# Complexity-ML/complexity-tokenizer

Hardware: AMD Instinct MI355X
Metric: MB/s raw UTF-8 encoded (encode_batch), 50k ByteLevel BPE, 1/2/4/8 MI355X (higher is better)
Workload: dtype u8

## Files before the change

complexity-tokenizer_amd/complexity_tokenizer/__init__.py:

```python
from __future__ import annotations

import ctypes
import gc
import os

import numpy as np

from . import _native as _n
from . import _fast

__version__ = "0.3.3"
__all__ = ["Tokenizer", "Trainer", "BpeTrainer", "WordPieceTrainer", "WordPieceModel", "UnigramTrainer", "UnigramModel", "Encoding",
           "BatchEncoding", "PanicException", "UnsupportedConfigError", "DeviceError", "__version__"]


class PanicException(BaseException):
    """Raised where the reference raises pyo3_runtime.PanicException (a Rust panic), e.g. a
    merge rank that indexes past the list of valid merges (reference src/bpe.rs:141)."""


class UnsupportedConfigError(NotImplementedError):
    """tokenizer.json selects a component outside the ByteLevel-BPE encode path."""


# ... 204 lines not shown
        return buf.raw[:n.value].decode("utf-8")

    @property
    def special_tokens(self) -> dict:
        out = {}
        for i in range(int(_n.lib.ctok_num_special_tokens(self._h))):
            n = ctypes.c_size_t()
            tid = ctypes.c_uint32()
            buf = ctypes.create_string_buffer(1024)
            rc = _n.lib.ctok_special_token(self._h, i, buf, 1024, ctypes.byref(n), ctypes.byref(tid))
            if rc != _n.CTOK_OK:
                _raise(rc)
            if n.value > 1024:
                buf = ctypes.create_string_buffer(n.value)
                _n.lib.ctok_special_token(self._h, i, buf, n.value, ctypes.byref(n), ctypes.byref(tid))
            out[buf.raw[:n.value].decode("utf-8")] = int(tid.value)
        return out

    def num_piece_added_tokens(self) -> int:
        return int(_n.lib.ctok_num_piece_added_tokens(self._h))

    @property
    def table_props(self) -> dict:
        tp = _n.TableProps(dev_mid_packed=-1)
        rc = _n.lib.ctok_get_table_props(self._h, int(self.device), ctypes.byref(tp))
        if rc != _n.CTOK_OK:
            _raise(rc)
        d = {k: None if getattr(tp, k) < 0 else bool(getattr(tp, k)) for k, _ in tp._fields_}
        d["dev_mid_packed"] = None if tp.dev_mid_packed < 0 else int(tp.dev_mid_packed)
        return d

    def encode_packed(self, text: np.ndarray, off: np.ndarray, timing: bool = False):
        text = np.ascontiguousarray(text, dtype=np.uint8)
        off = np.ascontiguousarray(off, dtype=np.uint64)
        n_docs = len(off) - 1
        if n_docs < 0:
            raise ValueError("offsets must hold n_docs + 1 entries")
        n_bytes = int(off[-1]) if n_docs >= 0 else 0
        if len(text) < n_bytes:
            raise ValueError("text shorter than offsets[-1]")
        cap = int(n_bytes + n_docs + 16)
        while True:
            ids = np.empty(max(cap, 1), dtype=np.uint32)
            tok_off = np.empty(n_docs + 1, dtype=np.uint64)
            ex = self._host_exec(timing)
            st = _n.Stats()
            rc = _n.lib.ctok_encode_batch(self._h, text.ctypes.data, off.ctypes.data, n_docs, ids.ctypes.data, cap,
                                          tok_off.ctypes.data, ctypes.byref(ex), ctypes.byref(st))
            if rc == _n.CTOK_E_CAPACITY:
                cap = int(tok_off[-1])
                continue
            if rc != _n.CTOK_OK:
# ... 470 lines not shown
```

complexity-tokenizer_amd/complexity_tokenizer/_native.py:

```python
from __future__ import annotations

import ctypes
import os

_HERE = os.path.dirname(os.path.abspath(__file__))
LIB_PATH = os.environ.get("CTOK_LIB", os.path.join(_HERE, "libctok.so"))

if not os.path.exists(LIB_PATH):
    raise ImportError(
        "complexity_tokenizer: native library not found at %s -- build it with "
        "`make -C complexity-tokenizer_amd/csrc` (or `python -c 'import __graft_entry__ as g; g.build()'`)" % LIB_PATH)


def _share_torch_hip_runtime():
    if os.environ.get("CTOK_NO_TORCH_HIP"):
        return
    try:
        import importlib.util
        spec = importlib.util.find_spec("torch")
    except (ImportError, ValueError):
        return
    if spec is None or not spec.origin:
        return
    path = os.path.join(os.path.dirname(spec.origin), "lib", "libamdhip64.so")
# ... 61 lines not shown
CTOK_P_PAD_LONGEST = 8
CTOK_P_PAD_TO_MAX = 16
CTOK_P_PAD_LEFT = 32
CTOK_P_PAD_ID = 64
CTOK_P_NO_POSTPROCESS = 128
CTOK_P_WINDOWS = 256
CTOK_PP_SEQUENCE = 0xFFFFFFFF


class PadOpts(ctypes.Structure):
    _fields_ = [("flags", ctypes.c_uint32), ("pad_id", ctypes.c_uint32), ("max_length", ctypes.c_uint64)]


class Tables(ctypes.Structure):
    _fields_ = [("vocab", ctypes.c_char_p), ("vocab_off", ctypes.c_void_p), ("vocab_id", ctypes.c_void_p),
                ("n_vocab", ctypes.c_uint64), ("merge_left", ctypes.c_void_p), ("merge_right", ctypes.c_void_p),
                ("n_merges", ctypes.c_uint64), ("added", ctypes.c_char_p), ("added_off", ctypes.c_void_p),
                ("added_id", ctypes.c_void_p), ("added_flags", ctypes.c_void_p), ("n_added", ctypes.c_uint64),
                ("nfc", ctypes.c_int), ("add_prefix_space", ctypes.c_int)]


class TableProps(ctypes.Structure):
    _fields_ = [(k, ctypes.c_int) for k in ("narrow", "compact", "short_packed", "ids16", "dev_narrow",
                                            "dev_short_packed", "last_rec16", "last_wire16", "dev_mid_packed")]


class TrainerConfig(ctypes.Structure):
    _fields_ = [("vocab_size", ctypes.c_uint64), ("min_frequency", ctypes.c_uint32),
                ("min_word_length", ctypes.c_uint64), ("inl_alpha", ctypes.c_float), ("inl_beta", ctypes.c_float),
                ("inl_gate", ctypes.c_float), ("inl_mu_target", ctypes.c_float),
                ("inl_velocity_max", ctypes.c_float), ("inl_beta_max", ctypes.c_float),
                ("special", ctypes.c_char_p), ("special_off", ctypes.POINTER(ctypes.c_uint64)),
                ("n_special", ctypes.c_uint64), ("device", ctypes.c_int)]


class TrainerCountStats(ctypes.Structure):
    _fields_ = [("pieces", ctypes.c_uint64), ("words", ctypes.c_uint64), ("unique_words", ctypes.c_uint64),
                ("chunks", ctypes.c_uint64), ("host_chunks", ctypes.c_uint64), ("rerun_chunks", ctypes.c_uint64),
                ("bytes_d2h", ctypes.c_uint64), ("ms_device", ctypes.c_double), ("ms_host", ctypes.c_double)]


class BpeTrainerConfig(ctypes.Structure):
    _fields_ = [("vocab_size", ctypes.c_uint64), ("min_frequency", ctypes.c_uint32),
                ("special", ctypes.c_char_p), ("special_off", ctypes.POINTER(ctypes.c_uint64)),
                ("n_special", ctypes.c_uint64), ("end_of_word_suffix", ctypes.c_char_p),
                ("continuing_subword_prefix", ctypes.c_char_p), ("show_progress", ctypes.c_int),
                ("device", ctypes.c_int)]
# ... 160 lines not shown
```

complexity-tokenizer_amd/csrc/ctok_encode.cpp:

```cpp
#include <chrono>
#include <cstdio>
#include <cstring>

#include "call_plan.h"
#include "gen/unicode_data.h"
#include "host_internal.h"
#include "knobs.h"

ctok::ctok() = default;
ctok::~ctok() = default;

namespace ctok_rt __attribute__((visibility("hidden"))) {

bool cp_fast_ok() {
  static const bool ok = [] {
    if (process_knobs().no_cp_ranges) return false;
    for (uint32_t cp = 0x3000; cp < 0x1F700; cp++) {
      const int rc = cp_range_class(cp);
      if (rc < 0) continue;
      const int cl = (ct_cls_stage2[ct_cls_stage1[cp >> 8] * 64 + ((cp & 255) >> 2)] >> ((cp & 3) * 2)) & 3;
      if (cl != rc || ct_nfc_stage2[ct_nfc_stage1[cp >> 8] * 256 + (cp & 255)] != 0) return false;
    }
    return true;
  }();
// ... 90 lines not shown
  tb.decomp_off = ds->decomp_off.p;
  tb.decomp_data = ds->decomp_data.p;
  tb.n_decomp = CT_DECOMP_N;
  tb.comp_key = ds->comp_key.p;
  tb.comp_val = ds->comp_val.p;
  tb.n_comp = CT_COMP_N;
  tb.bytemap_alnum = ds->alnum.p;
  tb.at_bytes = ds->at_bytes.p;
  tb.at_off = ds->at_off.p;
  tb.at_id = ds->at_id.p;
  tb.at_flags = ds->at_flags.p;
  tb.n_at = (uint32_t)t->at_id.size();
  const UploadKnobs knobs;
  tb.proper = (t->proper && !knobs.force_improper) ? 1 : 0;
  tb.compact = t->compact ? 1 : 0;
  tb.narrow = (t->narrow && !knobs.force_wide_slots) ? 1 : 0;
  tb.short_packed = (tb.narrow && t->short_packed && knobs.short_packed != 0) ? 1 : 0;
  {
    const int want = knobs.mid_packed;
    uint32_t v = (tb.narrow && tb.compact && t->short_packed && want > 0) ? (want >= 2 ? 2u : 1u) : 0u;
    if (v == 2 && !tb.short_packed) v = 1;
    tb.mid_packed = v;
  }
  tb.all_bytes = std::all_of(t->byte2id, t->byte2id + 256, [](int32_t v) { return v >= 0; }) ? 1 : 0;
  tb.dbg = knobs.dbg_mode;
  DeviceState* r = ds.get();
  t->devs[device] = std::move(ds);
  return r;
}

#define STEP(name, x)                                                                    \
  do {                                                                                   \
    HIPTRY(x);                                                                           \
    if (process_knobs().debug_sync) {                                                    \
      fprintf(stderr, "[ctok] %s launched\n", name);                                     \
      HIPTRY(hipStreamSynchronize(s));                                                   \
      fprintf(stderr, "[ctok] %s done\n", name);                                         \
    }                                                                                    \
  } while (0)

template <class Idle>
void spin_sync(DeviceState* ds, hipStream_t s, Idle idle) {
  HIPTRY(hipEventRecord(ds->ev_sync, s));
  for (;;) {
    hipError_t e = hipEventQuery(ds->ev_sync);
    if (e == hipSuccess) return;
// ... 556 lines not shown
```

complexity-tokenizer_amd/csrc/ctok_host.cpp:

```cpp
#include <emmintrin.h>

#include <cstdio>
#include <cstring>
#include <string_view>

#include "host_internal.h"
#include "knobs.h"
#include "window_hd.h"

namespace ctok_rt __attribute__((visibility("hidden"))) {

thread_local std::string g_err;


void check_offsets(const uint64_t* off, uint64_t n, const char* name) {
  if (off[0] != 0) throw_err(CTOK_E_ARG, std::string(name) + "[0] must be 0");
  for (uint64_t d = 0; d < n; d++)
    if (off[d + 1] < off[d]) throw_err(CTOK_E_ARG, std::string(name) + " must be non-decreasing");
}

struct DeviceCall {
  int dev;
  DeviceState* ds;
  std::lock_guard<std::recursive_mutex> lock;
// ... 395 lines not shown
    std::memcpy(off.data(), doc_off, (n_docs + 1) * 8);
  }
  if (bytes_d2h) *bytes_d2h = pbits.size() * 4 + (norm ? B + (n_docs + 1) * 8 : 0);
}

void pretokenize_device(ctok* t, int dev, const uint8_t* utf8, const uint64_t* doc_off, uint64_t n_docs,
                        const std::function<void(const DevicePretok&)>& use) {
  check_host_batch(utf8, doc_off, n_docs, "offsets");
  DeviceCall dc(t, dev);
  bool norm;
  use(pretokenize_staged(t, dc, utf8, doc_off, n_docs, &norm));
}
}


extern "C" {

const char* ctok_last_error(void) { return g_err.c_str(); }
const char* ctok_version(void) { return "0.3.3+mi355x.1"; }

int ctok_get_table_props(const ctok* tc, int device, ctok_table_props* out) {
  if (!tc || !out) return fail(CTOK_E_ARG, "null argument");
  ctok* t = const_cast<ctok*>(tc);
  *out = ctok_table_props{t->narrow, t->compact, t->short_packed, t->ids16, -1, -1, -1, -1, -1};
  std::lock_guard<std::mutex> lk(t->dev_mu);
  auto it = t->devs.find(device);
  if (it != t->devs.end()) {
    const DeviceState& ds = *it->second;
    out->dev_narrow = (int)ds.t.narrow;
    out->dev_short_packed = (int)ds.t.short_packed;
    out->last_rec16 = ds.last_rec16;
    out->last_wire16 = ds.last_wire16;
    out->dev_mid_packed = (int)ds.t.mid_packed;
  }
  return CTOK_OK;
}

int ctok_device_count(void) {
  int n = 0;
  if (hipGetDeviceCount(&n) != hipSuccess) return 0;
  return n;
}

int ctok_encode_batch_device(const ctok* tc, const uint8_t* d_utf8, const uint64_t* d_doc_off, uint64_t n_docs,
                             uint64_t n_bytes, uint32_t* d_ids, uint64_t ids_cap, uint64_t* d_tok_off,
                             uint64_t* n_tokens_out, const ctok_exec* exec, ctok_stats* stats) {
  if (!tc || !d_doc_off || !d_tok_off || (n_bytes && (!d_utf8 || !d_ids))) return fail(CTOK_E_ARG, "null argument");
  ctok* t = const_cast<ctok*>(tc);
  return run([&] {
    double t0 = now_ms();
    DeviceCall dc(t, exec);
    EncodeCall call;
    call.text = d_utf8, call.doc_off = d_doc_off, call.n_docs = n_docs, call.n_bytes = n_bytes;
    call.ids = d_ids, call.ids_cap = ids_cap, call.tok_off = d_tok_off;
    call.stream = dc.s, call.timing = dc.timing, call.stats = stats;
    uint64_t n = encode_device(t, dc.ds, call);
// ... 619 lines not shown
```

complexity-tokenizer_amd/csrc/ctok_internal.h:

```cpp
#pragma once
#include <hip/hip_runtime.h>

#include <cstdint>

#include "pair_tables_hd.h"

namespace ctok_dev {

constexpr uint32_t kErrPanic = 1u;

constexpr int kTileWords = 62;
constexpr int kTile = kTileWords * 64;
constexpr int kTileSlots = 4096;
constexpr int kSegWaves = 4;
constexpr int kSegUnroll = 4;
constexpr uint32_t kSegListBuf = 64 * kSegUnroll;
__host__ __device__ inline uint32_t seg_mark(uint32_t sl, uint32_t cls) { return sl | (cls << 12); }
__host__ __device__ inline uint32_t seg_mark_start(uint32_t m) { return m & 0xFFFu; }
__host__ __device__ inline uint32_t seg_mark_class(uint32_t m) { return m >> 12; }
constexpr int kShortMax = 32;
constexpr int kMedMax = 64;
constexpr uint32_t kCap0 = kTile, kCap1 = (kTile + 8) / 9, kCap2 = (kTile + 16) / 17, kCap3 = (kTile + 32) / 33;
constexpr uint32_t kCap0Lean = 1040;
constexpr int kNumClasses = 4;
constexpr int kNumCounters = 32;
constexpr int kC3Shards = 64;
constexpr int kCounterWords = kNumCounters + kC3Shards;
__host__ __device__ constexpr int ctr_stat(int c) { return c < 3 ? 6 + 2 * c : 16; }
__host__ __device__ constexpr int ctr_chunk(int c) { return c < 3 ? 13 + c : 18; }
constexpr int kCtrLong = 0;
constexpr int kCtrErr = 2;
constexpr int kCtrNfcDocs = 3;
constexpr int kCtrDropped = 4;
constexpr int kCtrPieces = 5;
constexpr int kCtrNfcFlag = 12;
constexpr int kCtrAnyMid = 19;
constexpr int kCtrAnyC3 = 20;
constexpr int kCtrEmptyDocs = 21;
constexpr int kCtrC3Count = 22;
constexpr int kCtrC3Take = 23;
constexpr uint32_t kC3SparseDefault = 65536;
constexpr uint32_t kWgRecWords = 4 * 1024 * 4;
constexpr int kMidPackedDefault = 2;
constexpr int kOverlapDefault = 1;
constexpr int kCtrSink = 31;
constexpr int kCtrOverflow = 25;
constexpr int kCtrLongIds = 26;
constexpr int kCtrLwWords = 27;
constexpr int kCtrRounds = 29;
constexpr int kLhBuckets = 65;
constexpr int kLhHist = 0, kLhScan = 80, kLhFill = 160, kLhTake = 240, kLhWords = 320;
__host__ __device__ inline uint32_t long_bucket(uint32_t n) { return n > 4096 ? 0u : 64u - (n - 1) / 64; }
__host__ __device__ inline uint32_t list_entry(uint32_t sl, uint32_t o, uint32_t n) { return sl | (o << 12) | (n << 24); }
__host__ __device__ inline uint32_t ent_len(uint32_t e) { return (e >> 24) & 127u; }
__host__ __device__ inline uint32_t ent_ord(uint32_t e) { return (e >> 12) & 0xFFFu; }
__host__ __device__ inline uint32_t long_ord(uint64_t e) { return (uint32_t)(e >> 32) & 0xFFFu; }
__host__ __device__ inline uint32_t long_len(uint64_t e) { return (uint32_t)(e >> 44) & 0x7FFFFu; }

constexpr uint32_t kRecLong = 0x40000000u, kRecLongMask = kRecLong - 1u;
constexpr uint32_t kRecMerged32 = 0xFFFFFFFFu, kRecMerged16 = 0xFFFFu;
__host__ __device__ inline uint32_t region_base(uint2 r, int cls) {
  return cls <= 0 ? 0u : cls == 1 ? (r.x & 0xFFFFu) : cls == 2 ? (r.x >> 16) : r.y;
}
__host__ __device__ inline uint32_t rec_short(uint32_t count, uint32_t sl) { return count | (sl << 16); }

// ... 28 lines not shown
  const uint8_t* cls_bmp;
  uint32_t cp_fast;
  const uint32_t* decomp_cp;
  const uint16_t* decomp_off;
  const uint32_t* decomp_data;
  uint32_t n_decomp;
  const uint64_t* comp_key;
  const uint32_t* comp_val;
  uint32_t n_comp;
  const uint8_t* bytemap_alnum;
  const uint8_t* at_bytes;
  const uint32_t* at_off;
  const uint32_t* at_id;
  const uint8_t* at_flags;
  uint32_t n_at;
  uint32_t proper;
  const uint32_t* eager;
  uint32_t window;
  const uint32_t* wmeta;
  uint32_t compact;
  uint32_t narrow;
  uint32_t short_packed;
  uint32_t mid_packed;
  uint32_t dbg;
  uint32_t all_bytes;
};

__host__ __device__ inline bool mid_folded(const Tables& t, uint32_t long_pieces) {
  return t.mid_packed == 2 && t.short_packed && t.n_at == 0 && long_pieces == 0;
}

struct Work {
  const uint8_t* text;
  uint32_t n_bytes;
  const uint64_t* doc_off;
  uint32_t n_docs;
  uint32_t* tfirst;
  uint32_t* pbits;
  uint32_t n_words;
  uint32_t n_tiles;
  uint32_t n_cus;
  uint32_t nfc_watch;
  uint32_t* nfc_bits;
  uint32_t mid_wide;
  uint32_t short_wgs;
  uint32_t chunk_sort;
// ... 162 lines not shown
```

complexity-tokenizer_amd/csrc/kernels.hip:

```cpp
#include "dev_common.h"
#include "pair_lookup_dev.h"

#include "chunk_sort_hd.h"
#include "merge_packed_hd.h"

namespace ctok_dev {


template <int K>
__device__ __forceinline__ uint32_t tile_share_init(const uint32_t* counts, uint32_t n_tiles, uint32_t t0,
                                                    uint32_t* s_pre, uint32_t* s_tsum, const uint2* tregion = nullptr,
                                                    int cls = -1, uint32_t* s_tbase = nullptr) {
  static_assert(K >= 1 && K <= 256 && (K & (K - 1)) == 0, "K: power of two <= 256");
  constexpr uint32_t kW = (K + 63) / 64;
  __shared__ uint32_t s_wsum[4];
  const uint32_t l = threadIdx.x, wv = l >> 6;
  const bool in = l < K && t0 + l < n_tiles;
  uint32_t c = 0, inc = 0;
  if (wv < kW) {
    c = in ? counts[t0 + l] : 0u;
    inc = wave_incl_scan(c);
    if (kW > 1 && (l & 63) == 63) s_wsum[wv] = inc;
  }
  if constexpr (kW > 1) __syncthreads();
// ... 287 lines not shown
        if (tid + (g + j) * NT < Es) {
          const uint32_t c = csort::code(N, mode, ent_len(e[j]));
          cr[g + j] = (c << 16) | atomicAdd(&S.bcnt[c], 1u);
        }
      }
    }
  }
  __syncthreads();
  if (tid < 64) {
    const uint32_t c = tid < csort::kMaxBuckets ? S.bcnt[tid] : 0u;
    const uint32_t inc = wave_incl_scan(c);
    if (tid < csort::kMaxBuckets) S.bfill[tid] = inc - c;
  }
  __syncthreads();
#pragma unroll
  for (uint32_t j = 0; j < EPT; j++) {
    const uint32_t q = tid + j * NT;
    if (q < Es) S.perm[S.bfill[cr[j] >> 16] + (cr[j] & 0xFFFFu)] = (uint16_t)q;
  }
  __syncthreads();
}

template <int N, bool COMPACT, bool HOT, uint32_t NT, uint32_t SORTCAP, bool L8 = false, int KT = 64, bool PK = false,
          bool LA = true, typename Load, int SKT>
__device__ __forceinline__ void class_pass(const Work& w, const Tables& t, const PairLds& P, const int32_t* s_b2id,
                                           PassLds<SORTCAP, SKT>& S, bool& loaded, Load&& load,
                                           lds_u32* s_key = nullptr, lds_u16* s_tok = nullptr) {
  using LC = LdsClass<N>;
  constexpr int K = KT;
  static_assert(KT <= (int)NT, "a thread per chunk tile");
  static_assert(KT <= SKT, "the shared scratch holds the pass's chunk");
  const uint32_t tid = threadIdx.x;
  uint32_t* err = &w.counters[kCtrErr];
  const uint32_t* list = class_list<N>(w);
  const uint32_t cap = class_cap<N>(w);
  const uint32_t* counts = w.tcls + (size_t)LC::cls * w.n_tiles;
  uint32_t st_bytes = 0, st_ids = 0;
  if (tid < 2) S.stat[tid] = 0;
  const uint32_t mode = w.chunk_sort;
  __syncthreads();
  uint32_t take = 1;
  const uint32_t U = w.unit;
  for (;;) {
    if (tid == 0) {
      S.chunk = atomicAdd(&w.counters[ctr_chunk(LC::cls)], take);
      S.take = take;
      S.next = 0;
// ... 54 lines not shown
      const uint32_t q = i < Es ? (uint32_t)S.perm[i] : i;
      kt = tile_of<K>(S.pre, q);
      return list[(size_t)(c0 + kt) * cap + (q - S.pre[kt])];
    };
    auto start_of = [&](uint32_t e, uint32_t kt) { return (c0 + kt) * kTile + (e & 0xFFFu); };
    auto body = [&](uint32_t e, uint32_t kt, const uint32_t* wv, auto&& hook) {
        const uint32_t tile = c0 + kt;
        const uint32_t s = tile * kTile + (e & 0xFFFu);
        const uint32_t o = ent_ord(e);
        const uint32_t n = ent_len(e);
        uint32_t pos = 0;
        auto out_of = [&](uint32_t mm) {
          pos = atomicAdd(&S.tsum[kt], mm);
          return w.scratch + (size_t)tile * kTileSlots + pos;
        };
        auto record = [&](uint32_t m) {
          CTOK_CHECK_REC(m >= 1 && m <= n && pos + m <= (uint32_t)kTileSlots && o < (uint32_t)kTileSlots,
                         "[ctok check] class pass N=%d PK=%d tile %u: record m=%u n=%u pos=%u ordinal=%u\n", N, (int)PK,
                         tile, m, n, pos, o);
          w.mrec[(size_t)tile * kTileSlots + o] = rec_short(m, pos);
          st_bytes += n;
          st_ids += m;
        };
        if constexpr (PK) {
          static_assert((N == 16 || N == 32) && L8 && COMPACT,
                        "the packed tiers are the 9..16 B and 17..32 B passes', ahead of merge_lds8, on compact tables");
          constexpr int ND = N / 2;
          uint32_t T[ND], R[ND], bytes[N];
          bool missing = false;
#pragma unroll
          for (int k = 0; k < N; k++) bytes[k] = byte_of(wv[k >> 2], k);
#pragma unroll
          for (int d = 0; d < ND; d++) {
            const int32_t i0 = s_b2id[bytes[2 * d]], i1 = s_b2id[bytes[2 * d + 1]];
            missing |= (((uint32_t)(2 * d) < n) & (i0 < 0)) | (((uint32_t)(2 * d + 1) < n) & (i1 < 0));
            T[d] = mpk::pack2((uint32_t)i0, (uint32_t)i1);
          }
          if (missing) {
            hook();
            defer_to_generic(w, s, o, n);
            return;
          }
          {
            uint32_t v[N];
#pragma unroll
            for (int k = 0; k < N - 1; k++) v[k] = t.pair0[(bytes[k] << 8) | bytes[k + 1]];
            v[N - 1] = kNoRank;
#pragma unroll
            for (int k = 0; k < N - 1; k++) v[k] = (uint32_t)k + 1 < n ? v[k] : kNoRank;
#pragma unroll
            for (int d = 0; d < ND; d++) R[d] = mpk::pack2(v[2 * d], v[2 * d + 1]);
          }
          uint32_t m = n;
          Lookup16<HOT> lk{t, P, err};
          if constexpr (N == 32) {
            bool more = mpk::tier(T, R, m, 16u, lk);
            uint32_t T8[8], R8[8];
            mpk::low_half(T, T8);
            mpk::low_half(R, R8);
            if (more) more = mpk::tier(T8, R8, m, 8u, lk);
            hook();
            if (more) {
              lds8_store_packed<0, 8, NT>(T8, R8, s_key, s_tok);
              m = merge_lds8_run<COMPACT, HOT, NT>(t, P, m, s_key, s_tok, err, out_of);
            } else if (m > 16) {
              store_packed_ids<0, N>(T, m, out_of(m));
            } else {
              store_packed_ids<0, 16>(T8, m, out_of(m));
            }
          } else {
            const bool more = mpk::tier(T, R, m, 8u, lk);
            hook();
            if (more) {
              lds8_store_packed<0, 8, NT>(T, R, s_key, s_tok);
              m = merge_lds8_run<COMPACT, HOT, NT>(t, P, m, s_key, s_tok, err, out_of);
            } else {
              store_packed_ids<0, N>(T, m, out_of(m));
            }
          }
          record(m);
          return;
        }
        uint32_t tk[N], rk[N];
        bool missing = false;
        {
#pragma unroll
          for (int k = 0; k < N; k++) {
            const int32_t id = s_b2id[byte_of(wv[k >> 2], k)];
            missing |= ((uint32_t)k < n) & (id < 0);
            tk[k] = (uint32_t)id;
          }
        }
        if (missing) {
          hook();
          defer_to_generic(w, s, o, n);
          return;
        }
        {
          uint32_t bytes[N];
#pragma unroll
          for (int k = 0; k < N; k++) bytes[k] = byte_of(wv[k >> 2], k);
// ... 125 lines not shown
  __syncthreads();
  if (tid == 0) {
    atomicAdd(&w.counters[ctr_stat(LC::cls)], S.stat[0]);
    atomicAdd(&w.counters[ctr_stat(LC::cls) + 1], S.stat[1]);
  }
  __syncthreads();
}


#ifndef CTOK_SHORT_NT
#define CTOK_SHORT_NT 1024
#endif
#ifndef CTOK_SHORT_SORTCAP
#define CTOK_SHORT_SORTCAP 7168
#endif
template <bool NARROW> struct ShortCfg {
  static constexpr uint32_t NT = NARROW ? CTOK_SHORT_NT : 1024;
  static constexpr uint32_t SORTCAP = NARROW ? CTOK_SHORT_SORTCAP : kSortCap;
};
constexpr int kShortKT = 64;

constexpr int kMidKT = 256;
constexpr uint32_t kFoldSortCut = 3 * (kMidKT - kShortKT) * 4 / 2;
template <bool COMPACT, bool NARROW, bool PK16 = false, bool PK32 = false>
__global__ __launch_bounds__(1024) void k_bpe_short(Work w, Tables t, uint32_t passes) {
  static_assert((NARROW && COMPACT) || !PK16, "the packed tier needs the narrow tables and compact values");
  static_assert(PK16 || !PK32, "the third pass is the packed instance's");
  if (w.report && blockIdx.x == 0 && threadIdx.x < 64) write_report(w);
  if (spec_failed(w)) return;
  constexpr uint32_t NT = ShortCfg<NARROW>::NT;
  constexpr uint32_t SORTCAP = ShortCfg<NARROW>::SORTCAP - (PK32 ? kFoldSortCut : 0u);
  extern __shared__ __attribute__((aligned(16))) uint4 s_img[];
  __shared__ int32_t s_b2id[256];
  __shared__ PassLds<SORTCAP, PK32 ? kMidKT : kShortKT> S;
  __shared__ uint32_t s_key[NARROW ? 8 * NT : 1];
  __shared__ uint16_t s_tok[NARROW ? 8 * NT : 1];
  const uint32_t tid = threadIdx.x;
  const uint4* img = NARROW ? t.lds16_image : t.lds_image;
  auto load = [&] {
    for (uint32_t i = tid; i < kLdsImageBytes / 16; i += NT) s_img[i] = img[i];
    for (uint32_t i = tid; i < 256; i += NT) s_b2id[i] = t.byte2id[i];
  };
  bool loaded = false;
  const PairLds P{(const lds_u64*)s_img, (const lds_u32*)(s_img + kHotBuckets)};
  lds_u32* sk = (lds_u32*)s_key;
  lds_u16* st = (lds_u16*)s_tok;
  WgRec::begin(w.wgrec, 0);
  if (passes & 1u)
    class_pass<8, COMPACT, true, NT, SORTCAP, NARROW, kShortKT>(w, t, P, s_b2id, S, loaded, load, sk, st);
  if (passes & 2u)
    class_pass<16, COMPACT, true, NT, SORTCAP, NARROW, kShortKT, PK16>(w, t, P, s_b2id, S, loaded, load, sk, st);
  if constexpr (PK32) {
    if (passes & 4u) {
      if (tid == 0) S.next = (mid_folded(t, w.counters[kCtrLong]) && w.counters[kCtrAnyMid] != 0) ? 1u : 0u;
      __syncthreads();
      const uint32_t fold = S.next;
      if (fold)
        class_pass<32, COMPACT, true, NT, SORTCAP, NARROW, kMidKT, true, false>(w, t, P, s_b2id, S, loaded, load, sk, st);
    }
  }
  WgRec::end(w.wgrec, 0, loaded ? 1u : 0u);
}


template <bool COMPACT, bool NARROW>
__device__ __forceinline__ uint32_t merge_wave64(const Tables& t, const PairLds& P, uint32_t& tok, uint32_t rk,
                                                 uint64_t& lv, uint32_t* err) {
  const uint32_t lane = threadIdx.x & 63;
  for (;;) {
    const uint32_t best = wave_min_full_u32((rk << 6) | lane);
    const uint32_t r = best >> 6, bi = best & 63u;
    if (r == kNoRank) break;
    const uint32_t nid = COMPACT ? r : uni(t.rank_newid[r]);
    const uint64_t right = lv & ~((2ull << bi) - 1ull);
    const uint32_t p = (uint32_t)__builtin_ctzll(right);
    const uint64_t after = right & (right - 1ull);
    const bool has_r = after != 0;
    const uint32_t q = has_r ? (uint32_t)__builtin_ctzll(after) : 0u;
    const uint64_t left = lv & ((1ull << bi) - 1ull);
    const bool has_l = left != 0;
    const uint32_t pv = has_l ? 63u - (uint32_t)__builtin_clzll(left) : 0u;
// ... 66 lines not shown

constexpr int kSparseWaves = 16;

template <bool COMPACT, bool NARROW>
__global__ __launch_bounds__(64 * kSparseWaves) void k_bpe_sparse(Work w, Tables t, uint32_t n) {
  if (spec_failed(w)) return;
  WgRec::begin(w.wgrec, 3);
  extern __shared__ __attribute__((aligned(16))) uint4 s_dyn[];
  __shared__ int32_t s_b2id[256];
  const uint32_t tid = threadIdx.x;
  const uint4* img = NARROW ? t.lds16_image : t.lds_image;
  for (uint32_t i = tid; i < kLdsImageBytes / 16; i += 64 * kSparseWaves) s_dyn[i] = img[i];
  for (uint32_t i = tid; i < 256; i += 64 * kSparseWaves) s_b2id[i] = t.byte2id[i];
  __syncthreads();
  const PairLds P{(const lds_u64*)s_dyn, (const lds_u32*)(s_dyn + kHotBuckets)};
  sparse_c3<COMPACT, NARROW>(w, t, P, s_b2id, n);
  __syncthreads();
  WgRec::end(w.wgrec, 3, 1);
}


template <int CLS> struct MidCfg { static constexpr int KT = kMidKT; };

template <bool COMPACT, int CLS, bool NARROW, uint32_t NT = 512, bool PK = false>
__global__ __launch_bounds__(NT) void k_bpe_mid(Work w, Tables t) {
  static_assert(!PK || (CLS == 2 && NARROW && COMPACT), "the packed tiers need the narrow tables and compact values");
  if (spec_failed(w)) return;
  constexpr int KT = MidCfg<CLS>::KT;
  extern __shared__ __attribute__((aligned(16))) uint4 s_img[];
  __shared__ int32_t s_b2id[256];
  __shared__ PassLds<kSortCap, KT> S;
  __shared__ uint32_t s_key[NARROW ? 8 * NT : 1];
  __shared__ uint16_t s_tok[NARROW ? 8 * NT : 1];
  if constexpr (CLS == 2) WgRec::begin(w.wgrec, 1);
  if (w.counters[CLS == 2 ? kCtrAnyMid : kCtrAnyC3] == 0) {
    if constexpr (CLS == 2) WgRec::end(w.wgrec, 1, 0);
    return;
  }
  __shared__ uint32_t s_left;
  if (threadIdx.x == 0)
    s_left = (uint64_t)__atomic_load_n(&w.counters[ctr_chunk(CLS)], __ATOMIC_RELAXED) * w.unit < w.n_tiles;
  __syncthreads();
  if (!s_left) {
    if constexpr (CLS == 2) WgRec::end(w.wgrec, 1, 0);
    return;
  }
  const uint32_t tid = threadIdx.x;
  const uint4* img = NARROW ? t.lds16_image : t.lds_image;
  for (uint32_t i = tid; i < kLdsImageBytes / 16; i += NT) s_img[i] = img[i];
  for (uint32_t i = tid; i < 256; i += NT) s_b2id[i] = t.byte2id[i];
  bool loaded = true;
  const PairLds P{(const lds_u64*)s_img, (const lds_u32*)(s_img + kHotBuckets)};
  class_pass<CLS == 2 ? 32 : 64, COMPACT, true, NT, kSortCap, NARROW, KT, PK>(w, t, P, s_b2id, S, loaded, [] {},
                                                                             (lds_u32*)s_key, (lds_u16*)s_tok);
  if constexpr (CLS == 2) WgRec::end(w.wgrec, 1, 1);
}

template <bool C, int CLS, bool NW, bool PK = false>
static hipError_t launch_mid_t(const Work& w, const Tables& t, hipStream_t s, const Lx& x) {
  static LdsAttr attr;
  HIPCHK(lds_attr_once(attr, (const void*)k_bpe_mid<C, CLS, NW, 512, PK>, kLdsImageBytes));
  if (!w.n_tiles) return hipSuccess;
  const uint32_t grid = min((w.n_tiles + w.unit - 1) / w.unit, w.n_cus);
  if constexpr (CLS == 2) {
    if (w.mid_wide) {
      static LdsAttr attr768;
      HIPCHK(lds_attr_once(attr768, (const void*)k_bpe_mid<C, CLS, NW, 768, PK>, kLdsImageBytes));
      launch_lx(x, k_bpe_mid<C, CLS, NW, 768, PK>, grid, 768, kLdsImageBytes, s, w, t);
      return hipGetLastError();
    }
  }
  launch_lx(x, k_bpe_mid<C, CLS, NW, 512, PK>, grid, 512, kLdsImageBytes, s, w, t);
  return hipGetLastError();
}
template <bool C, int CLS>
static hipError_t launch_mid(const Work& w, const Tables& t, hipStream_t s, const Lx& x = {}) {
  if constexpr (C && CLS == 2) {
    if (t.narrow && t.mid_packed) return launch_mid_t<true, 2, true, true>(w, t, s, x);
  }
  return t.narrow ? launch_mid_t<C, CLS, true>(w, t, s, x) : launch_mid_t<C, CLS, false>(w, t, s, x);
}

template <bool C, bool NW, bool PK = false, bool PK32 = false>
static hipError_t launch_short_t(const Work& w, const Tables& t, hipStream_t s, const Lx& x) {
  static LdsAttr attr;
  HIPCHK(lds_attr_once(attr, (const void*)k_bpe_short<C, NW, PK, PK32>, kLdsImageBytes));
  if (!w.n_tiles) return hipSuccess;
  const uint32_t grid = min((w.n_tiles + w.unit - 1) / w.unit, w.short_wgs ? min(w.short_wgs, w.n_cus) : w.n_cus);
  if (t.dbg == 30) {
    const uint32_t last = PK32 ? 4u : 2u;
    for (uint32_t pass = 1u; pass <= last; pass <<= 1)
      launch_lx(Lx{pass == 1u ? x.start : nullptr, pass == last ? x.stop : nullptr}, k_bpe_short<C, NW, PK, PK32>, grid,
                ShortCfg<NW>::NT, kLdsImageBytes, s, w, t, pass);
  } else {
    launch_lx(x, k_bpe_short<C, NW, PK, PK32>, grid, ShortCfg<NW>::NT, kLdsImageBytes, s, w, t, PK32 ? 7u : 3u);
  }
  return hipGetLastError();
}
template <bool C>
static hipError_t launch_short(const Work& w, const Tables& t, hipStream_t s, const Lx& x) {
  if constexpr (C) {
    if (t.narrow && t.short_packed && t.mid_packed == 2) return launch_short_t<true, true, true, true>(w, t, s, x);
    if (t.narrow && t.short_packed) return launch_short_t<true, true, true>(w, t, s, x);
  }
  return t.narrow ? launch_short_t<C, true>(w, t, s, x) : launch_short_t<C, false>(w, t, s, x);
}

template <bool C, bool NW>
static hipError_t launch_sparse_t(const Work& w, const Tables& t, uint32_t n_pieces, hipStream_t s, const Lx& x) {
  static LdsAttr attr;
  HIPCHK(lds_attr_once(attr, (const void*)k_bpe_sparse<C, NW>, kLdsImageBytes));
  const uint32_t grid = std::max(1u, std::min((n_pieces + kSparseWaves - 1) / kSparseWaves, w.n_cus));
  launch_lx(x, k_bpe_sparse<C, NW>, grid, 64 * kSparseWaves, kLdsImageBytes, s, w, t, n_pieces);
  return hipGetLastError();
}

hipError_t launch_c3_sparse(const Work& w, const Tables& t, uint32_t n_pieces, hipStream_t s, Lx x) {
  if (!n_pieces || n_pieces > w.c3_max || !w.n_tiles) return hipSuccess;
  if (t.compact)
    return t.narrow ? launch_sparse_t<true, true>(w, t, n_pieces, s, x) : launch_sparse_t<true, false>(w, t, n_pieces, s, x);
  return t.narrow ? launch_sparse_t<false, true>(w, t, n_pieces, s, x) : launch_sparse_t<false, false>(w, t, n_pieces, s, x);
}

hipError_t launch_bpe_class(const Work& w, const Tables& t, int cls, hipStream_t s, Lx x) {
// ... 20 lines not shown
```

complexity-tokenizer_amd/csrc/knobs.h:

```cpp
#pragma once
#include <cstdint>
#include <cstdlib>
#include <optional>

#include "chunk_sort_hd.h"
#include "ctok_internal.h"
#include "table_compile.h"

namespace ctok_rt __attribute__((visibility("hidden"))) {

inline bool env_set(const char* name) { return getenv(name) != nullptr; }
inline int env_int(const char* name, int dflt) {
  const char* v = getenv(name);
  return v ? atoi(v) : dflt;
}
inline std::optional<uint64_t> env_u64(const char* name) {
  const char* v = getenv(name);
  return v ? std::optional<uint64_t>(strtoull(v, nullptr, 10)) : std::nullopt;
}

struct LoadKnobs {
  bool load_timing = env_set("CTOK_LOAD_TIMING");
  TableOptions tables = [] {
    TableOptions o;
    o.force_wide = env_set("CTOK_FORCE_WIDE");
    o.no_hot_table = env_set("CTOK_NO_HOT_TABLE");
    o.no_window = env_set("CTOK_NO_WINDOW");
    o.no_piece_table = env_set("CTOK_NO_PIECE_TABLE");
    o.merge_slack = (size_t)env_int("CTOK_MERGE_SLACK", (int)o.merge_slack);
    o.merge16_slack = (size_t)env_int("CTOK_MERGE16_SLACK", (int)o.merge16_slack);
    o.piece_slack = (size_t)env_int("CTOK_PIECE_SLACK", (int)o.piece_slack);
    return o;
  }();
};

struct UploadKnobs {
  bool force_improper = env_set("CTOK_FORCE_IMPROPER");
  bool force_wide_slots = env_set("CTOK_FORCE_WIDE_SLOTS");
  int short_packed = env_int("CTOK_SHORT_PACKED", 1);
  int mid_packed = env_int("CTOK_MID_PACKED", ctok_dev::kMidPackedDefault);
  uint32_t dbg_mode = (uint32_t)env_int("CTOK_DBG_MODE", 0);
};

struct ProcessKnobs {
  bool no_cp_ranges = env_set("CTOK_NO_CP_RANGES");
  bool debug_sync = env_set("CTOK_DEBUG_SYNC");
  bool safe_capacities = env_set("CTOK_SAFE_CAPACITIES");
  bool hostprof = env_set("CTOK_HOSTPROF");
  uint32_t unit = (uint32_t)env_int("CTOK_UNIT", 0);
  bool rec32 = env_set("CTOK_REC32");
  bool wgrec = env_set("CTOK_WGREC");
  bool stamps = env_set("CTOK_STAMPS");
  bool copy_results = env_set("CTOK_COPY_RESULTS");
  bool no_chunk_ramp = env_set("CTOK_NO_CHUNK_RAMP");
  bool pipe_trace = env_set("CTOK_PIPE_TRACE");
};
inline const ProcessKnobs& process_knobs() {
  static const ProcessKnobs k;
  return k;
}

struct CallKnobs {
  bool no_nfc_speculation = env_set("CTOK_NO_NFC_SPECULATION");
// ... 20 lines not shown
```

complexity-tokenizer_amd/csrc/merge_packed_hd.h:

```cpp
#pragma once
#include <cstdint>

#if defined(__HIPCC__)
#define MPK_HD __host__ __device__ __forceinline__
#define MPK_UNROLL _Pragma("unroll")
#else
#define MPK_HD inline
#define MPK_UNROLL
#endif

namespace mpk {

constexpr uint32_t kNone = 0xFFFFu;

MPK_HD uint32_t shr16(uint32_t hi, uint32_t lo) {
#if defined(__HIP_DEVICE_COMPILE__)
  return __builtin_amdgcn_alignbyte(hi, lo, 2u);
#else
  return (lo >> 16) | (hi << 16);
#endif
}
MPK_HD uint32_t umin(uint32_t a, uint32_t b) { return a < b ? a : b; }
MPK_HD uint32_t pack2(uint32_t lo, uint32_t hi) { return (lo & 0xFFFFu) | (hi << 16); }
MPK_HD uint32_t bfi(uint32_t mask, uint32_t a, uint32_t b) { return (a & mask) | (b & ~mask); }

template <int K, int ND>
MPK_HD uint32_t half(const uint32_t (&A)[ND]) {
  static_assert(K >= 0 && K < 2 * ND, "slot within the array");
  return (K & 1) ? A[K >> 1] >> 16 : A[K >> 1] & 0xFFFFu;
}
template <int ND>
MPK_HD uint32_t min_key(const uint32_t (&R)[ND]) {
  uint32_t key = ~0u;
MPK_UNROLL
  for (int d = 0; d < ND; d++) {
    key = umin(key, (R[d] << 16) | (uint32_t)(2 * d));
    key = umin(key, (R[d] & 0xFFFF0000u) | (uint32_t)(2 * d + 1));
  }
  return key;
}

template <int ND, class LK>
MPK_HD bool step(uint32_t (&T)[ND], uint32_t (&R)[ND], uint32_t& m, LK& lk) {
  static_assert(ND == 8 || ND == 16, "16 or 32 slots: the slot is the key's low 4 or 5 bits");
  const uint32_t key = min_key(R);
  const uint32_t best = key >> 16, bi = key & (uint32_t)(2 * ND - 1);
  if (best == kNone) return false;
  const uint32_t nid = lk.new_id(best) & 0xFFFFu;
  const uint32_t D = bi >> 1;
  const bool odd = (bi & 1u) != 0;
  uint32_t S[ND];
MPK_UNROLL
  for (int d = 0; d < ND; d++) S[d] = shr16(d + 1 < ND ? T[d + 1] : ~0u, T[d]);
  uint32_t A[ND + 1];
  A[0] = odd ? T[0] : 0u;
MPK_UNROLL
  for (int d = 1; d < ND; d++) A[d] = odd ? T[d] : S[d - 1];
  A[ND] = odd ? ~0u : S[ND - 1];
  uint32_t L0 = 0, R0 = 0;
MPK_UNROLL
  for (int d = 0; d < ND; d++) {
    L0 = D == (uint32_t)d ? A[d] : L0;
    R0 = D == (uint32_t)d ? A[d + 1] : R0;
  }
  const uint32_t L = L0 & 0xFFFFu, Rt = R0 >> 16;
  const bool has_l = bi > 0, has_r = bi + 2 < m;
  lk.start(L, nid, Rt, has_l, has_r);
// ... 5 lines not shown
    const bool right = bi < (uint32_t)(2 * d + 1);
    T[d] = D == (uint32_t)d ? Y : (right ? S[d] : T[d]);
    const uint32_t sr = shr16(d + 1 < ND ? R[d + 1] : ~0u, R[d]);
    R[d] = right ? sr : R[d];
    mask[d] = D == (uint32_t)d ? mA : (D == (uint32_t)(d + 1) ? mB : 0u);
  }
  m--;
  uint32_t rl, rr;
  lk.finish(rl, rr);
  const uint32_t vv = odd ? pack2(rl, rr) : pack2(rr, rl);
MPK_UNROLL
  for (int d = 0; d < ND; d++) R[d] = bfi(mask[d], vv, R[d]);
  return true;
}

template <int ND, class LK>
MPK_HD bool tier(uint32_t (&T)[ND], uint32_t (&R)[ND], uint32_t& m, uint32_t stop, LK& lk) {
  for (;;) {
    if (m <= stop) return true;
    if (!step(T, R, m, lk)) return false;
  }
}

MPK_HD void low_half(const uint32_t (&A)[16], uint32_t (&lo)[8]) {
MPK_UNROLL
  for (int d = 0; d < 8; d++) lo[d] = A[d];
}

template <int K, int ND>
MPK_HD uint32_t lds8_key(const uint32_t (&R)[ND]) {
  static_assert(K < 8, "a slot of the 8-slot tier");
  const uint32_t r = half<K>(R);
  return r == kNone ? ~0u : (r << 3) | (uint32_t)K;
}

}
```

include/ctok.h:

```cpp
#ifndef CTOK_H
#define CTOK_H

#include <stddef.h>
#include <stdint.h>

#ifdef __cplusplus
extern "C" {
#endif

typedef struct ctok ctok;

enum {
  CTOK_OK = 0,
  CTOK_E_IO = -1,
  CTOK_E_PARSE = -2,
  CTOK_E_UNSUPPORTED = -3,
  CTOK_E_ARG = -4,
  CTOK_E_CAPACITY = -5,
  CTOK_E_PANIC = -6,
  CTOK_E_DEVICE = -7,
  CTOK_E_NOTFOUND = -8
};

const char* ctok_last_error(void);
// ... 22 lines not shown
  const uint32_t* added_id;
  const uint8_t* added_flags;
  uint64_t n_added;
  int nfc;
  int add_prefix_space;
} ctok_tables;
int ctok_create_from_tables(const ctok_tables* tables, ctok** out);
void ctok_destroy(ctok* tok);

uint64_t ctok_vocab_size(const ctok* tok);
int ctok_token_to_id(const ctok* tok, const char* token, size_t len, uint32_t* id);
int ctok_id_to_token(const ctok* tok, uint32_t id, char* buf, size_t cap, size_t* len);
uint64_t ctok_num_special_tokens(const ctok* tok);
int ctok_special_token(const ctok* tok, uint64_t i, char* buf, size_t cap, size_t* len, uint32_t* id);

uint64_t ctok_num_piece_added_tokens(const ctok* tok);
int ctok_piece_can_contain(const uint8_t* raw, size_t len);

typedef struct ctok_table_props {
  int narrow, compact, short_packed, ids16;
  int dev_narrow, dev_short_packed;
  int last_rec16, last_wire16;
  int dev_mid_packed;
} ctok_table_props;
int ctok_get_table_props(const ctok* tok, int device, ctok_table_props* out);

typedef struct ctok_exec {
  int device;
  void* stream;
  uint32_t flags;
  const int* devices;
  int n_devices;
  uint32_t chunk_mb;
  uint32_t host_threads;
} ctok_exec;

#define CTOK_F_TIMING 1u

typedef struct ctok_stats {
  double ms_total;
  double ms_device;
  double ms_pretok;
  double ms_bpe_short;
  double ms_bpe_long;
  double ms_emit;
  double ms_h2d, ms_d2h;
// ... 103 lines not shown
```

Baseline: 178,300.

## Finish BPE merges for words of 8 bytes or fewer in registers, dropping merge_lds8

Adds a packed 8-slot tier that completes the final merge stage for pieces of up to 8 bytes in per-thread registers (mpk::run on 4-word arrays), instead of staging keys through LDS and running merge_lds8_run. It is on by default (CTOK_PK8=1) for narrow packed tables. This lets the short and mid kernels drop their s_key and s_tok LDS arrays and the reduced sort-capacity cut, freeing LDS and perhaps allowing more occupancy. The cost is a serial per-thread merge loop that may raise register use and cause divergence.

```diff
diff --git a/complexity-tokenizer_amd/complexity_tokenizer/__init__.py b/complexity-tokenizer_amd/complexity_tokenizer/__init__.py
--- a/complexity-tokenizer_amd/complexity_tokenizer/__init__.py
+++ b/complexity-tokenizer_amd/complexity_tokenizer/__init__.py
@@ -250,12 +250,13 @@
 
     @property
     def table_props(self) -> dict:
-        tp = _n.TableProps(dev_mid_packed=-1)
+        tp = _n.TableProps(dev_mid_packed=-1, dev_pk8=-1)
         rc = _n.lib.ctok_get_table_props(self._h, int(self.device), ctypes.byref(tp))
         if rc != _n.CTOK_OK:
             _raise(rc)
         d = {k: None if getattr(tp, k) < 0 else bool(getattr(tp, k)) for k, _ in tp._fields_}
         d["dev_mid_packed"] = None if tp.dev_mid_packed < 0 else int(tp.dev_mid_packed)
+        d["dev_pk8"] = None if tp.dev_pk8 < 0 else int(tp.dev_pk8)
         return d
 
     def encode_packed(self, text: np.ndarray, off: np.ndarray, timing: bool = False):
diff --git a/complexity-tokenizer_amd/complexity_tokenizer/_native.py b/complexity-tokenizer_amd/complexity_tokenizer/_native.py
--- a/complexity-tokenizer_amd/complexity_tokenizer/_native.py
+++ b/complexity-tokenizer_amd/complexity_tokenizer/_native.py
@@ -107,7 +107,8 @@
 
 class TableProps(ctypes.Structure):
     _fields_ = [(k, ctypes.c_int) for k in ("narrow", "compact", "short_packed", "ids16", "dev_narrow",
-                                            "dev_short_packed", "last_rec16", "last_wire16", "dev_mid_packed")]
+                                            "dev_short_packed", "last_rec16", "last_wire16", "dev_mid_packed",
+                                            "dev_pk8")]
 
 
 class TrainerConfig(ctypes.Structure):
diff --git a/complexity-tokenizer_amd/csrc/ctok_encode.cpp b/complexity-tokenizer_amd/csrc/ctok_encode.cpp
--- a/complexity-tokenizer_amd/csrc/ctok_encode.cpp
+++ b/complexity-tokenizer_amd/csrc/ctok_encode.cpp
@@ -136,6 +136,7 @@
     if (v == 2 && !tb.short_packed) v = 1;
     tb.mid_packed = v;
   }
+  tb.pk8 = ((tb.short_packed || tb.mid_packed) && knobs.pk8 != 0) ? 1 : 0;
   tb.all_bytes = std::all_of(t->byte2id, t->byte2id + 256, [](int32_t v) { return v >= 0; }) ? 1 : 0;
   tb.dbg = knobs.dbg_mode;
   DeviceState* r = ds.get();
diff --git a/complexity-tokenizer_amd/csrc/ctok_host.cpp b/complexity-tokenizer_amd/csrc/ctok_host.cpp
--- a/complexity-tokenizer_amd/csrc/ctok_host.cpp
+++ b/complexity-tokenizer_amd/csrc/ctok_host.cpp
@@ -441,7 +441,7 @@
 int ctok_get_table_props(const ctok* tc, int device, ctok_table_props* out) {
   if (!tc || !out) return fail(CTOK_E_ARG, "null argument");
   ctok* t = const_cast<ctok*>(tc);
-  *out = ctok_table_props{t->narrow, t->compact, t->short_packed, t->ids16, -1, -1, -1, -1, -1};
+  *out = ctok_table_props{t->narrow, t->compact, t->short_packed, t->ids16, -1, -1, -1, -1, -1, -1};
   std::lock_guard<std::mutex> lk(t->dev_mu);
   auto it = t->devs.find(device);
   if (it != t->devs.end()) {
@@ -451,6 +451,7 @@
     out->last_rec16 = ds.last_rec16;
     out->last_wire16 = ds.last_wire16;
     out->dev_mid_packed = (int)ds.t.mid_packed;
+    out->dev_pk8 = (int)ds.t.pk8;
   }
   return CTOK_OK;
 }
diff --git a/complexity-tokenizer_amd/csrc/ctok_internal.h b/complexity-tokenizer_amd/csrc/ctok_internal.h
--- a/complexity-tokenizer_amd/csrc/ctok_internal.h
+++ b/complexity-tokenizer_amd/csrc/ctok_internal.h
@@ -41,6 +41,7 @@
 constexpr int kCtrC3Take = 23;
 constexpr uint32_t kC3SparseDefault = 65536;
 constexpr uint32_t kWgRecWords = 4 * 1024 * 4;
+constexpr int kPk8Default = 1;
 constexpr int kMidPackedDefault = 2;
 constexpr int kOverlapDefault = 1;
 constexpr int kCtrSink = 31;
@@ -115,6 +116,7 @@
   uint32_t narrow;
   uint32_t short_packed;
   uint32_t mid_packed;
+  uint32_t pk8;
   uint32_t dbg;
   uint32_t all_bytes;
 };
diff --git a/complexity-tokenizer_amd/csrc/kernels.hip b/complexity-tokenizer_amd/csrc/kernels.hip
--- a/complexity-tokenizer_amd/csrc/kernels.hip
+++ b/complexity-tokenizer_amd/csrc/kernels.hip
@@ -333,7 +333,7 @@
 }
 
 template <int N, bool COMPACT, bool HOT, uint32_t NT, uint32_t SORTCAP, bool L8 = false, int KT = 64, bool PK = false,
-          bool LA = true, typename Load, int SKT>
+          bool LA = true, bool PK8 = false, typename Load, int SKT>
 __device__ __forceinline__ void class_pass(const Work& w, const Tables& t, const PairLds& P, const int32_t* s_b2id,
                                            PassLds<SORTCAP, SKT>& S, bool& loaded, Load&& load,
                                            lds_u32* s_key = nullptr, lds_u16* s_tok = nullptr) {
@@ -434,9 +434,10 @@
           st_bytes += n;
           st_ids += m;
         };
-        if constexpr (PK) {
-          static_assert((N == 16 || N == 32) && L8 && COMPACT,
-                        "the packed tiers are the 9..16 B and 17..32 B passes', ahead of merge_lds8, on compact tables");
+        if constexpr (PK || (PK8 && N == 8)) {
+          static_assert((N == 16 || N == 32 || (N == 8 && PK8)) && L8 && COMPACT,
+                        "the packed tiers are the 9..16 B and 17..32 B passes', ahead of merge_lds8, on compact tables; "
+                        "with the packed 8-slot tier, the <= 8 B pass's too");
           constexpr int ND = N / 2;
           uint32_t T[ND], R[ND], bytes[N];
           bool missing = false;
@@ -471,24 +472,48 @@
             mpk::low_half(T, T8);
             mpk::low_half(R, R8);
             if (more) more = mpk::tier(T8, R8, m, 8u, lk);
+            uint32_t T4[4], R4[4];
+            if constexpr (PK8) {
+              mpk::low_half(T8, T4);
+              mpk::low_half(R8, R4);
+              if (more) mpk::run(T4, R4, m, lk);
+            }
             hook();
             if (more) {
-              lds8_store_packed<0, 8, NT>(T8, R8, s_key, s_tok);
-              m = merge_lds8_run<COMPACT, HOT, NT>(t, P, m, s_key, s_tok, err, out_of);
+              if constexpr (PK8) {
+                store_packed_ids<0, 8>(T4, m, out_of(m));
+              } else {
+                lds8_store_packed<0, 8, NT>(T8, R8, s_key, s_tok);
+                m = merge_lds8_run<COMPACT, HOT, NT>(t, P, m, s_key, s_tok, err, out_of);
+              }
             } else if (m > 16) {
               store_packed_ids<0, N>(T, m, out_of(m));
             } else {
               store_packed_ids<0, 16>(T8, m, out_of(m));
             }
-          } else {
+          } else if constexpr (N == 16) {
             const bool more = mpk::tier(T, R, m, 8u, lk);
+            uint32_t T4[4], R4[4];
+            if constexpr (PK8) {
+              mpk::low_half(T, T4);
+              mpk::low_half(R, R4);
+              if (more) mpk::run(T4, R4, m, lk);
+            }
             hook();
             if (more) {
-              lds8_store_packed<0, 8, NT>(T, R, s_key, s_tok);
-              m = merge_lds8_run<COMPACT, HOT, NT>(t, P, m, s_key, s_tok, err, out_of);
+              if constexpr (PK8) {
+                store_packed_ids<0, 8>(T4, m, out_of(m));
+              } else {
+                lds8_store_packed<0, 8, NT>(T, R, s_key, s_tok);
+                m = merge_lds8_run<COMPACT, HOT, NT>(t, P, m, s_key, s_tok, err, out_of);
+              }
             } else {
               store_packed_ids<0, N>(T, m, out_of(m));
             }
+          } else {
+            mpk::run(T, R, m, lk);
+            hook();
+            store_packed_ids<0, N>(T, m, out_of(m));
           }
           record(m);
           return;
@@ -660,19 +685,27 @@
 
 constexpr int kMidKT = 256;
 constexpr uint32_t kFoldSortCut = 3 * (kMidKT - kShortKT) * 4 / 2;
-template <bool COMPACT, bool NARROW, bool PK16 = false, bool PK32 = false>
+template <bool COMPACT, bool NARROW, bool PK16 = false, bool PK32 = false, bool PK8 = false>
 __global__ __launch_bounds__(1024) void k_bpe_short(Work w, Tables t, uint32_t passes) {
   static_assert((NARROW && COMPACT) || !PK16, "the packed tier needs the narrow tables and compact values");
   static_assert(PK16 || !PK32, "the third pass is the packed instance's");
+  static_assert(PK16 || !PK8, "the packed 8-slot tier is the packed instances'");
   if (w.report && blockIdx.x == 0 && threadIdx.x < 64) write_report(w);
   if (spec_failed(w)) return;
   constexpr uint32_t NT = ShortCfg<NARROW>::NT;
-  constexpr uint32_t SORTCAP = ShortCfg<NARROW>::SORTCAP - (PK32 ? kFoldSortCut : 0u);
+  constexpr bool LDS8 = NARROW && !PK8;
+  constexpr uint32_t SORTCAP = ShortCfg<NARROW>::SORTCAP - (PK32 && LDS8 ? kFoldSortCut : 0u);
   extern __shared__ __attribute__((aligned(16))) uint4 s_img[];
   __shared__ int32_t s_b2id[256];
   __shared__ PassLds<SORTCAP, PK32 ? kMidKT : kShortKT> S;
-  __shared__ uint32_t s_key[NARROW ? 8 * NT : 1];
-  __shared__ uint16_t s_tok[NARROW ? 8 * NT : 1];
+  lds_u32* sk = nullptr;
+  lds_u16* st = nullptr;
+  if constexpr (LDS8) {
+    __shared__ uint32_t s_key[8 * NT];
+    __shared__ uint16_t s_tok[8 * NT];
+    sk = (lds_u32*)s_key;
+    st = (lds_u16*)s_tok;
+  }
   const uint32_t tid = threadIdx.x;
   const uint4* img = NARROW ? t.lds16_image : t.lds_image;
   auto load = [&] {
@@ -681,20 +714,18 @@
   };
   bool loaded = false;
   const PairLds P{(const lds_u64*)s_img, (const lds_u32*)(s_img + kHotBuckets)};
-  lds_u32* sk = (lds_u32*)s_key;
-  lds_u16* st = (lds_u16*)s_tok;
   WgRec::begin(w.wgrec, 0);
   if (passes & 1u)
-    class_pass<8, COMPACT, true, NT, SORTCAP, NARROW, kShortKT>(w, t, P, s_b2id, S, loaded, load, sk, st);
+    class_pass<8, COMPACT, true, NT, SORTCAP, NARROW, kShortKT, false, true, PK8>(w, t, P, s_b2id, S, loaded, load, sk, st);
   if (passes & 2u)
-    class_pass<16, COMPACT, true, NT, SORTCAP, NARROW, kShortKT, PK16>(w, t, P, s_b2id, S, loaded, load, sk, st);
+    class_pass<16, COMPACT, true, NT, SORTCAP, NARROW, kShortKT, PK16, true, PK8>(w, t, P, s_b2id, S, loaded, load, sk, st);
   if constexpr (PK32) {
     if (passes & 4u) {
       if (tid == 0) S.next = (mid_folded(t, w.counters[kCtrLong]) && w.counters[kCtrAnyMid] != 0) ? 1u : 0u;
       __syncthreads();
       const uint32_t fold = S.next;
       if (fold)
-        class_pass<32, COMPACT, true, NT, SORTCAP, NARROW, kMidKT, true, false>(w, t, P, s_b2id, S, loaded, load, sk, st);
+        class_pass<32, COMPACT, true, NT, SORTCAP, NARROW, kMidKT, true, false, PK8>(w, t, P, s_b2id, S, loaded, load, sk, st);
     }
   }
   WgRec::end(w.wgrec, 0, loaded ? 1u : 0u);
@@ -807,16 +838,23 @@
 
 template <int CLS> struct MidCfg { static constexpr int KT = kMidKT; };
 
-template <bool COMPACT, int CLS, bool NARROW, uint32_t NT = 512, bool PK = false>
+template <bool COMPACT, int CLS, bool NARROW, uint32_t NT = 512, bool PK = false, bool PK8 = false>
 __global__ __launch_bounds__(NT) void k_bpe_mid(Work w, Tables t) {
   static_assert(!PK || (CLS == 2 && NARROW && COMPACT), "the packed tiers need the narrow tables and compact values");
+  static_assert(PK || !PK8, "the packed 8-slot tier is the packed instance's");
   if (spec_failed(w)) return;
   constexpr int KT = MidCfg<CLS>::KT;
   extern __shared__ __attribute__((aligned(16))) uint4 s_img[];
   __shared__ int32_t s_b2id[256];
   __shared__ PassLds<kSortCap, KT> S;
-  __shared__ uint32_t s_key[NARROW ? 8 * NT : 1];
-  __shared__ uint16_t s_tok[NARROW ? 8 * NT : 1];
+  lds_u32* sk = nullptr;
+  lds_u16* st = nullptr;
+  if constexpr (NARROW && !PK8) {
+    __shared__ uint32_t s_key[8 * NT];
+    __shared__ uint16_t s_tok[8 * NT];
+    sk = (lds_u32*)s_key;
+    st = (lds_u16*)s_tok;
+  }
   if constexpr (CLS == 2) WgRec::begin(w.wgrec, 1);
   if (w.counters[CLS == 2 ? kCtrAnyMid : kCtrAnyC3] == 0) {
     if constexpr (CLS == 2) WgRec::end(w.wgrec, 1, 0);
@@ -836,55 +874,60 @@
   for (uint32_t i = tid; i < 256; i += NT) s_b2id[i] = t.byte2id[i];
   bool loaded = true;
   const PairLds P{(const lds_u64*)s_img, (const lds_u32*)(s_img + kHotBuckets)};
-  class_pass<CLS == 2 ? 32 : 64, COMPACT, true, NT, kSortCap, NARROW, KT, PK>(w, t, P, s_b2id, S, loaded, [] {},
-                                                                             (lds_u32*)s_key, (lds_u16*)s_tok);
+  class_pass<CLS == 2 ? 32 : 64, COMPACT, true, NT, kSortCap, NARROW, KT, PK, true, PK8>(w, t, P, s_b2id, S, loaded,
+                                                                                        [] {}, sk, st);
   if constexpr (CLS == 2) WgRec::end(w.wgrec, 1, 1);
 }
 
-template <bool C, int CLS, bool NW, bool PK = false>
+template <bool C, int CLS, bool NW, bool PK = false, bool PK8 = false>
 static hipError_t launch_mid_t(const Work& w, const Tables& t, hipStream_t s, const Lx& x) {
   static LdsAttr attr;
-  HIPCHK(lds_attr_once(attr, (const void*)k_bpe_mid<C, CLS, NW, 512, PK>, kLdsImageBytes));
+  HIPCHK(lds_attr_once(attr, (const void*)k_bpe_mid<C, CLS, NW, 512, PK, PK8>, kLdsImageBytes));
   if (!w.n_tiles) return hipSuccess;
   const uint32_t grid = min((w.n_tiles + w.unit - 1) / w.unit, w.n_cus);
   if constexpr (CLS == 2) {
     if (w.mid_wide) {
       static LdsAttr attr768;
-      HIPCHK(lds_attr_once(attr768, (const void*)k_bpe_mid<C, CLS, NW, 768, PK>, kLdsImageBytes));
-      launch_lx(x, k_bpe_mid<C, CLS, NW, 768, PK>, grid, 768, kLdsImageBytes, s, w, t);
+      HIPCHK(lds_attr_once(attr768, (const void*)k_bpe_mid<C, CLS, NW, 768, PK, PK8>, kLdsImageBytes));
+      launch_lx(x, k_bpe_mid<C, CLS, NW, 768, PK, PK8>, grid, 768, kLdsImageBytes, s, w, t);
       return hipGetLastError();
     }
   }
-  launch_lx(x, k_bpe_mid<C, CLS, NW, 512, PK>, grid, 512, kLdsImageBytes, s, w, t);
+  launch_lx(x, k_bpe_mid<C, CLS, NW, 512, PK, PK8>, grid, 512, kLdsImageBytes, s, w, t);
   return hipGetLastError();
 }
 template <bool C, int CLS>
 static hipError_t launch_mid(const Work& w, const Tables& t, hipStream_t s, const Lx& x = {}) {
   if constexpr (C && CLS == 2) {
+    if (t.narrow && t.mid_packed && t.pk8) return launch_mid_t<true, 2, true, true, true>(w, t, s, x);
     if (t.narrow && t.mid_packed) return launch_mid_t<true, 2, true, true>(w, t, s, x);
   }
   return t.narrow ? launch_mid_t<C, CLS, true>(w, t, s, x) : launch_mid_t<C, CLS, false>(w, t, s, x);
 }
 
-template <bool C, bool NW, bool PK = false, bool PK32 = false>
+template <bool C, bool NW, bool PK = false, bool PK32 = false, bool PK8 = false>
 static hipError_t launch_short_t(const Work& w, const Tables& t, hipStream_t s, const Lx& x) {
   static LdsAttr attr;
-  HIPCHK(lds_attr_once(attr, (const void*)k_bpe_short<C, NW, PK, PK32>, kLdsImageBytes));
+  HIPCHK(lds_attr_once(attr, (const void*)k_bpe_short<C, NW, PK, PK32, PK8>, kLdsImageBytes));
   if (!w.n_tiles) return hipSuccess;
   const uint32_t grid = min((w.n_tiles + w.unit - 1) / w.unit, w.short_wgs ? min(w.short_wgs, w.n_cus) : w.n_cus);
   if (t.dbg == 30) {
     const uint32_t last = PK32 ? 4u : 2u;
     for (uint32_t pass = 1u; pass <= last; pass <<= 1)
-      launch_lx(Lx{pass == 1u ? x.start : nullptr, pass == last ? x.stop : nullptr}, k_bpe_short<C, NW, PK, PK32>, grid,
+      launch_lx(Lx{pass == 1u ? x.start : nullptr, pass == last ? x.stop : nullptr}, k_bpe_short<C, NW, PK, PK32, PK8>, grid,
                 ShortCfg<NW>::NT, kLdsImageBytes, s, w, t, pass);
   } else {
-    launch_lx(x, k_bpe_short<C, NW, PK, PK32>, grid, ShortCfg<NW>::NT, kLdsImageBytes, s, w, t, PK32 ? 7u : 3u);
+    launch_lx(x, k_bpe_short<C, NW, PK, PK32, PK8>, grid, ShortCfg<NW>::NT, kLdsImageBytes, s, w, t, PK32 ? 7u : 3u);
   }
   return hipGetLastError();
 }
 template <bool C>
 static hipError_t launch_short(const Work& w, const Tables& t, hipStream_t s, const Lx& x) {
   if constexpr (C) {
+    if (t.narrow && t.short_packed && t.pk8) {
+      if (t.mid_packed == 2) return launch_short_t<true, true, true, true, true>(w, t, s, x);
+      return launch_short_t<true, true, true, false, true>(w, t, s, x);
+    }
     if (t.narrow && t.short_packed && t.mid_packed == 2) return launch_short_t<true, true, true, true>(w, t, s, x);
     if (t.narrow && t.short_packed) return launch_short_t<true, true, true>(w, t, s, x);
   }
diff --git a/complexity-tokenizer_amd/csrc/knobs.h b/complexity-tokenizer_amd/csrc/knobs.h
--- a/complexity-tokenizer_amd/csrc/knobs.h
+++ b/complexity-tokenizer_amd/csrc/knobs.h
@@ -39,6 +39,7 @@
   bool force_wide_slots = env_set("CTOK_FORCE_WIDE_SLOTS");
   int short_packed = env_int("CTOK_SHORT_PACKED", 1);
   int mid_packed = env_int("CTOK_MID_PACKED", ctok_dev::kMidPackedDefault);
+  int pk8 = env_int("CTOK_PK8", ctok_dev::kPk8Default);
   uint32_t dbg_mode = (uint32_t)env_int("CTOK_DBG_MODE", 0);
 };
 
diff --git a/complexity-tokenizer_amd/csrc/merge_packed_hd.h b/complexity-tokenizer_amd/csrc/merge_packed_hd.h
--- a/complexity-tokenizer_amd/csrc/merge_packed_hd.h
+++ b/complexity-tokenizer_amd/csrc/merge_packed_hd.h
@@ -42,7 +42,7 @@
 
 template <int ND, class LK>
 MPK_HD bool step(uint32_t (&T)[ND], uint32_t (&R)[ND], uint32_t& m, LK& lk) {
-  static_assert(ND == 8 || ND == 16, "16 or 32 slots: the slot is the key's low 4 or 5 bits");
+  static_assert(ND == 4 || ND == 8 || ND == 16, "8, 16 or 32 slots: the slot is the key's low 3, 4 or 5 bits");
   const uint32_t key = min_key(R);
   const uint32_t best = key >> 16, bi = key & (uint32_t)(2 * ND - 1);
   if (best == kNone) return false;
@@ -94,9 +94,15 @@
   }
 }
 
-MPK_HD void low_half(const uint32_t (&A)[16], uint32_t (&lo)[8]) {
+template <int ND, class LK>
+MPK_HD void run(uint32_t (&T)[ND], uint32_t (&R)[ND], uint32_t& m, LK& lk) {
+  while (step(T, R, m, lk)) {}
+}
+
+template <int NH>
+MPK_HD void low_half(const uint32_t (&A)[2 * NH], uint32_t (&lo)[NH]) {
 MPK_UNROLL
-  for (int d = 0; d < 8; d++) lo[d] = A[d];
+  for (int d = 0; d < NH; d++) lo[d] = A[d];
 }
 
 template <int K, int ND>
diff --git a/include/ctok.h b/include/ctok.h
--- a/include/ctok.h
+++ b/include/ctok.h
@@ -68,6 +68,7 @@
   int dev_narrow, dev_short_packed;
   int last_rec16, last_wire16;
   int dev_mid_packed;
+  int dev_pk8;
 } ctok_table_props;
 int ctok_get_table_props(const ctok* tok, int device, ctok_table_props* out);
 
```

Result: no change. 179,700, median of 6 (+0.8%).
